# epam/Zstandard

Hardware: AMD Instinct MI355X
Metric: GiB/s compress @ level 3, 64 KiB chunks (higher is better)
Workload: dtype u8; 1 GPU; 4096 independent 65536 B chunks per GPU per step, level 3, BASELINE config[1] shape (Silesia unavailable offline -> Zipf-token log stream, SURVEY 8d); chunks_per_gpu=4096, chunk_bytes=65536, level=3, parallelism=chunks sharded over 1 GPU(s), no collective in the data path

## Files before the change

zstandard_amd/csrc/lz_kernels.hip:

```cpp
#include "zsmi_device.h"
#include "zsmi_scratch.h"
#include <type_traits>

#ifndef ZS_CAND_G
#define ZS_CAND_G 8
#endif
#ifndef ZS_CAND_G_BIG
#define ZS_CAND_G_BIG 16
#endif
#define ZS_CAND_GOF(TLOG) ((TLOG) > ZS_TABLE_LOG_SMALL ? ZS_CAND_G_BIG : ZS_CAND_G)
#ifndef ZS_CAND_DEPTH
#define ZS_CAND_DEPTH 2
#endif
#define ZS_CAND_WAVES(NT) (3 * (NT))
#define ZS_CAND_ROW 65u
#define ZS_CAND_LDS(TLOG, NT) ((size_t)(NT) * (4u << (TLOG)) + 3u * (NT) * ZS_CAND_GOF(TLOG) * ZS_CAND_ROW * 4u + (NT) * 256u + 3u * 16u * 8u + 32u)
#define ZS_SLOT_EMPTY 0xFFFFFFFFu
__device__ __forceinline__ uint32_t zs_hash_short(uint32_t lo, uint32_t hi) { return __umul24(lo, 0x9E3779u) + __umul24(__builtin_amdgcn_alignbit(hi, lo, 16), 0x85EBCBu); }
__device__ __forceinline__ uint32_t zs_hash_long(uint32_t lo, uint32_t hi)
{ return __umul24(lo, 0x9E3779u) + __umul24(__builtin_amdgcn_alignbit(hi, lo, 24), 0x85EBCBu) + __umul24(hi >> 16, 0xC2B2AFu); }

template <int TLOG, int NT, bool PFX = false>
__global__ void __launch_bounds__(64 * ZS_CAND_WAVES(NT))
k_lz_candidates(const uint8_t *__restrict__ src, const ZsUnitDesc *__restrict__ units, uint32_t block0,
                uint16_t *__restrict__ distAll, uint8_t *__restrict__ distHiAll, uint32_t *__restrict__ candCount,
                const ZsCDictEntry *__restrict__ dictTab = nullptr, const uint32_t *__restrict__ unitDict = nullptr,
                const uint32_t *__restrict__ liveUnits = nullptr)
{
    static_assert(!PFX || TLOG == ZS_TABLE_LOG_BIG, "a prefixed unit spans up to 128 KiB of positions");
    if (liveUnits && blockIdx.x >= *liveUnits) return;
    const uint32_t *dictImg = nullptr; uint32_t pfx = 0;
    if constexpr (PFX) {
        const ZsCDictEntry &de = dictTab[unitDict ? unitDict[blockIdx.x] : 0u];
        dictImg = de.img; pfx = (uint32_t)__builtin_amdgcn_readfirstlane((int)de.pfx);
    }
    extern __shared__ __attribute__((aligned(16))) uint32_t candLds[];
    constexpr bool BIG = TLOG > ZS_TABLE_LOG_SMALL;
    constexpr uint32_t G = ZS_CAND_GOF(TLOG), GP = G * 64u, H = G / NT;
    constexpr uint32_t M = ZS_CAND_DEPTH;
    constexpr uint32_t LPS = 64u / G;
    constexpr uint32_t WD = G / 4u + 2u;
    static_assert(G == 8 || G == 16, "a hasher lane takes G consecutive positions of a group: 8 or 16");
    const uint32_t wave = (uint32_t)__builtin_amdgcn_readfirstlane((int)(threadIdx.x >> 6)), lane = threadIdx.x & 63u;
    const uint32_t tab = (wave < NT) ? wave : ((wave < 2 * NT) ? wave - NT : wave - 2 * NT);
    uint32_t *T = candLds + ((size_t)tab << TLOG);
    uint32_t *opnd = candLds + ((size_t)NT << TLOG);
    constexpr uint32_t ROW = ZS_CAND_ROW, GR = G * ROW;
    constexpr uint32_t RING = 3u * NT * GR;
    uint64_t *runMarks = reinterpret_cast<uint64_t *>(opnd + RING + NT * 64u);
    uint32_t *runFlag = opnd + RING + NT * 64u + 3u * 16u * 2u;
    const ZsUnitDesc ud = units[blockIdx.x];
    const uint8_t *s = src + ud.srcOff;
    const uint32_t n = ud.size;
    const size_t slot = (size_t)(ud.firstBlock - block0);
    uint16_t *dist = zs_block_dist(distAll, slot);
    uint8_t *distHi = zs_block_dist_hi(distHiAll, slot);
    const uint32_t hashable = (n >= 8) ? n - 7 : 0;
    const uint32_t nGroups = (hashable + GP - 1) / GP;
    if (threadIdx.x < 2) zs_block_cand(candCount, slot, threadIdx.x) = 0;
    if (nGroups == 0) return;
    if (n >= 16 && (n & 15u) == 0) {
        uint4 f;
        __builtin_memcpy(&f, s, 16);
        const uint32_t splat = (f.x & 0xFFu) * 0x01010101u;
        if (((f.x ^ splat) | (f.y ^ splat) | (f.z ^ splat) | (f.w ^ splat)) == 0) {
            if (threadIdx.x == 0) candLds[0] = 0;
            __syncthreads();
            uint32_t mixed = 0;
            for (uint32_t i = threadIdx.x * 16u; i < n && !mixed; i += ZS_CAND_WAVES(NT) * 64u * 16u) {
                uint4 v;
                __builtin_memcpy(&v, s + i, 16);
                mixed = (v.x ^ splat) | (v.y ^ splat) | (v.z ^ splat) | (v.w ^ splat);
            }
            if (mixed) candLds[0] = 1u;
            __syncthreads();
            const bool uniform = candLds[0] == 0;
            __syncthreads();
            if (uniform) return;
        }
    }
    const uint32_t dummyBase = ((uint32_t)(NT - tab) << TLOG) + RING + tab * 64u;
    auto mergeRead = [&](uint32_t g, uint32_t (&mS)[H], uint32_t (&mL)[H]) {
        const uint32_t *xb = opnd + (size_t)(g % 3u) * NT * GR + (NT > 1 ? tab * H : 0u) * ROW + lane;
        #pragma unroll
        for (uint32_t uu = 0; uu < H; uu++) { mS[uu] = xb[uu * ROW]; mL[uu] = (NT > 1) ? xb[GR + uu * ROW] : 0u; }
    };
    uint32_t found = 0;
    const uint32_t matchlessBelow = n >> ZS_MATCHLESS_SHIFT;
    auto mergeStore = [&](uint32_t g, const uint32_t (&mS)[H], const uint32_t (&mL)[H]) {
        const uint32_t sbase = g * GP + ((NT > 1) ? tab * H * 64u : 0u);
        uint64_t hiMine = 0;
        #pragma unroll
        for (uint32_t uu = 0; uu < H; uu++) {
            const uint32_t dm = (NT > 1) ? (mL[uu] ? mL[uu] : mS[uu]) : mS[uu];
            if (BIG) { const uint64_t hi = __ballot((dm >> 16) != 0); if (lane == uu) hiMine = hi; }
            if (found < matchlessBelow) {
                if ((g + 1u) * GP <= hashable) found += (uint32_t)__popcll(__ballot(dm != 0));
                else found += (uint32_t)__popcll(__ballot(dm != 0 && sbase + uu * 64 + lane < hashable));
            }
            dist[sbase + uu * 64 + lane] = (uint16_t)dm;
        }
        if (BIG && lane < H) *reinterpret_cast<uint64_t *>(distHi + ((sbase + lane * 64) >> 3)) = hiMine;
    };
    if (wave >= 2 * NT) {
        __syncthreads(); __syncthreads();
        for (uint32_t i = 2; i <= nGroups + 1; i++) {
            uint32_t mS[H], mL[H];
            mergeRead(i - 2, mS, mL);
            if (__builtin_amdgcn_readfirstlane((int)runFlag[((i - 2) % 3u) * 2u + tab])) {
                if (lane == 0) runFlag[((i - 2) % 3u) * 2u + tab] = 0;
                #pragma unroll
                for (uint32_t uu = 0; uu < H; uu++) {
                    const uint64_t marks = runMarks[((i - 2) % 3u) * 16u + ((NT > 1) ? tab * H : 0u) + uu];
                    if ((marks >> lane) & 1ull) { if (NT > 1) mL[uu] = 1u; else mS[uu] = 1u; }
                }
            }
            mergeStore(i - 2, mS, mL);
            __syncthreads();
        }
        if (lane == 0) zs_block_cand(candCount, slot, tab) = found;
        return;
    }

    if (wave < NT) {
        if constexpr (PFX) {
            uint4 *t4 = reinterpret_cast<uint4 *>(T);
            const uint4 *img4 = reinterpret_cast<const uint4 *>(dictImg + ((size_t)tab << TLOG));
            #pragma unroll 8
            for (uint32_t i = lane; i < (1u << TLOG) / 4; i += 64) t4[i] = img4[i];
        } else {
            uint4 *t4 = reinterpret_cast<uint4 *>(T);
            const uint4 e = make_uint4(ZS_SLOT_EMPTY, ZS_SLOT_EMPTY, ZS_SLOT_EMPTY, ZS_SLOT_EMPTY);
            #pragma unroll 8
            for (uint32_t i = lane; i < (1u << TLOG) / 4; i += 64) t4[i] = e;
        }
        uint32_t ringSlot = 0;
        __syncthreads();
        for (uint32_t i = 1; i <= nGroups; i++) {
            uint32_t *ob = opnd + ((size_t)ringSlot * NT + tab) * GR + lane;
            const uint32_t base = (i - 1) * GP + lane + (PFX ? pfx : 0u);
            uint32_t op[G], entry[G], old[G];
            #pragma unroll
            for (uint32_t u = 0; u < G; u++) op[u] = ob[u * ROW];
            #pragma unroll
            for (uint32_t u = 0; u < G; u++) {
                uint32_t pu = base + u * 64u;
                asm volatile("" : "+v"(pu));
                entry[u] = (op[u] & 0xFFFE0000u) | pu;
                old[u] = atomicExch(&T[op[u] & 0xFFFFu], entry[u]);
            }
            #pragma unroll
            for (uint32_t u = 0; u < G; u++) {
                const uint32_t x = old[u] ^ entry[u], dd = entry[u] - old[u];
                ob[u * ROW] = (max(x, dd) < (1u << 17)) ? dd : 0u;
            }
            ringSlot = (ringSlot == 2u) ? 0u : ringSlot + 1u;
            __syncthreads();
        }
        __syncthreads();
        return;
    }

    auto run = [&](auto roleTag) {
        constexpr bool LONG = decltype(roleTag)::value;
        const uint32_t stepOfLane = lane / LPS, l0 = (lane % LPS) * G;
        const uint32_t wbase = stepOfLane * ROW + l0;
        const uint32_t last8 = n - 8;
        auto loadGroup = [&](uint32_t g, uint32_t (&w)[WD]) {
            const uint32_t o = g * GP + lane * G;
            #pragma unroll
            for (uint32_t k = 0; k < WD / 2; k++) {
                const uint32_t ok = o + 8u * k, oc = min(ok, last8);
                const uint64_t v = zs_load64(s + oc) >> (8u * min(ok - oc, 7u));
                w[2 * k] = (uint32_t)v; w[2 * k + 1] = (uint32_t)(v >> 32);
            }
        };
        uint32_t bufA[M][WD], bufB[M][WD];
        auto loadM = [&](uint32_t g0, uint32_t (&buf)[M][WD]) {
            #pragma unroll
            for (uint32_t k = 0; k < M; k++) loadGroup(min(g0 + k, nGroups), buf[k]);
        };
        auto iter = [&](auto wholeTag, uint32_t i, const uint32_t (&w)[WD]) {
            constexpr bool WHOLE = decltype(wholeTag)::value;
            const uint32_t ringSlot = i % 3u;
            if (i < nGroups) {
                uint32_t *ob = opnd + ((size_t)ringSlot * NT + tab) * GR + wbase;
                const uint32_t pbase = i * GP + lane * G;
                #pragma unroll
                for (uint32_t u = 0; u < G; u++) {
                    const uint32_t k = u >> 2, sh = u & 3u;
                    const uint32_t lo = sh ? __builtin_amdgcn_alignbyte(w[k + 1], w[k], sh) : w[k];
                    const uint32_t hi = sh ? __builtin_amdgcn_alignbyte(w[min(k + 2, WD - 1)], w[k + 1], sh) : w[k + 1];
                    uint32_t h = LONG ? zs_hash_long(lo, hi) : zs_hash_short(lo, hi);
                    asm volatile("" : "+v"(h));
                    const uint32_t r = __builtin_amdgcn_alignbit(h, h, 32 - TLOG);
                    ob[u] = (WHOLE || pbase + u < hashable) ? (r & (0xFFFE0000u | ((1u << TLOG) - 1u))) : ((r & 0xFFFE0000u) | (dummyBase + l0 + u));
                }
                bool flat = false;
                uint64_t flatLanes = 0;
                if (WHOLE && __ballot(w[0] == w[1])) {
                    uint32_t diff = w[0] ^ __builtin_amdgcn_alignbyte(w[0], w[0], 1);
                    #pragma unroll
                    for (uint32_t k = 1; k < WD; k++) diff |= w[k] ^ w[k - 1];
                    flat = diff == 0;
                    flatLanes = __ballot(flat);
                }
                if (flatLanes) {
                    const uint32_t key = flat ? ((w[0] & 0xFFu) | 0x100u) : 0u;
                    const uint32_t keyBelow = (uint32_t)__builtin_amdgcn_update_dpp(0, (int)key, 0x138, 0xF, 0xF, true);
                    const uint32_t keyAbove = (uint32_t)__builtin_amdgcn_update_dpp(0, (int)key, 0x130, 0xF, 0xF, true);
                    const bool markFirst = flat && keyBelow == key && (lane % LPS) != 0u;
                    const bool innerLast = flat && keyAbove == key && (lane % LPS) != LPS - 1u;
                    if (flat) {
                        uint32_t h = LONG ? zs_hash_long(w[0], w[1]) : zs_hash_short(w[0], w[1]);
                        asm volatile("" : "+v"(h));
                        const uint32_t away = (__builtin_amdgcn_alignbit(h, h, 32 - TLOG) & 0xFFFE0000u) | (dummyBase + l0);
                        if (markFirst) ob[0] = away;
                        #pragma unroll
                        for (uint32_t u = 1; u + 1 < G; u++) ob[u] = away + u;
                        if (innerLast) ob[G - 1] = away + (G - 1);
                    }
                    if (!LONG) {
                        if (lane < NT) runFlag[ringSlot * 2u + lane] = 1u;
                        const uint32_t bits = flat ? (((1u << G) - 2u) | (markFirst ? 1u : 0u)) : 0u;
                        if (G == 8) reinterpret_cast<uint8_t *>(runMarks + ringSlot * 16u)[lane] = (uint8_t)bits;
                        else reinterpret_cast<uint16_t *>(runMarks + ringSlot * 16u)[lane] = (uint16_t)bits;
                    }
                }
            }
            __syncthreads();
        };
        auto step = [&](uint32_t i, const uint32_t (&w)[WD]) {
            if (i > nGroups + 1) return;
            if ((i + 1) * GP + 8u <= n) iter(std::true_type{}, i, w); else iter(std::false_type{}, i, w);
        };
        if (!LONG && lane < 6u) runFlag[lane] = 0;
        loadM(0, bufA);
        for (uint32_t g0 = 0; g0 <= nGroups + 1; g0 += 2 * M) {
            loadM(g0 + M, bufB);
            #pragma unroll
            for (uint32_t k = 0; k < M; k++) step(g0 + k, bufA[k]);
            loadM(g0 + 2 * M, bufA);
            #pragma unroll
            for (uint32_t k = 0; k < M; k++) step(g0 + M + k, bufB[k]);
        }
    };
    if (tab == 0) run(std::false_type{}); else run(std::true_type{});
}

__global__ void __launch_bounds__(1024)
k_lz_dict_tables(const ZsCDictEntry entry, ZsCDictEntry *__restrict__ entryOut)
{
    constexpr int TLOG = ZS_TABLE_LOG_BIG;
    __shared__ uint32_t T[1u << TLOG];
    const uint32_t tab = blockIdx.x, tid = threadIdx.x;
    const uint8_t *__restrict__ pre = entry.pre; const uint32_t pfx = entry.pfx; uint32_t *__restrict__ img = const_cast<uint32_t *>(entry.img);
    if (tab == 0 && tid == 0) *entryOut = entry;
    for (uint32_t i = tid; i < (1u << TLOG); i += 1024) T[i] = 0;
    __syncthreads();
    const uint32_t hashable = pfx >= 8 ? pfx - 7 : 0;
    for (uint32_t p = tid; p < hashable; p += 1024) {
        const uint64_t v = zs_load64(pre + p);
        const uint32_t lo = (uint32_t)v, hi = (uint32_t)(v >> 32);
        const uint32_t h = tab ? zs_hash_long(lo, hi) : zs_hash_short(lo, hi);
        const uint32_t r = __builtin_amdgcn_alignbit(h, h, 32 - TLOG);
        atomicMax(&T[r & ((1u << TLOG) - 1u)], ((p + 1u) << 15) | (r >> 17));
    }
    __syncthreads();
    uint32_t *out = img + ((size_t)tab << TLOG);
    for (uint32_t i = tid; i < (1u << TLOG); i += 1024) {
        const uint32_t k = T[i];
        out[i] = k ? (((k & 0x7FFFu) << 17) | ((k >> 15) - 1u)) : ZS_SLOT_EMPTY;
    }
}

#ifndef ZS_WALK_MINW
#define ZS_WALK_MINW 1
#endif
#define ZS_WALK_WGRP(WLOG) ((WLOG) >= 9 ? 4 : 2)
#ifndef ZS_WALK_LPW_256
#define ZS_WALK_LPW_256 2
#endif
#ifndef ZS_WALK_LPW_512
#define ZS_WALK_LPW_512 4
#endif
#define ZS_WALK_LPW(WLOG) ((WLOG) >= 9 ? ZS_WALK_LPW_512 : ZS_WALK_LPW_256)
#define ZS_WALK_THREADS(BIG, WLOG) ((((BIG) ? ZS_UNIT_MAX : ZS_BLOCK_MAX) >> (WLOG)) * ZS_WALK_LPW(WLOG))
#define ZS_WALK_KERNEL(LOOK, REPW, BIG, WLOG) k_lz_walk<ZS_WALK_LPW(WLOG), ZS_WALK_WGRP(WLOG), LOOK, REPW, BIG, ZS_WALK_THREADS(BIG, WLOG)>
#ifndef ZS_WALK_SKEW
#define ZS_WALK_SKEW  24u
#endif
#define ZS_WALK_FRONT 48u
#define ZS_WALK_TAIL  144u
#define ZS_WALK_SRCBYTES(CAPB) ((((CAPB) + ZS_WALK_TAIL + ZS_WALK_SKEW * (((CAPB) + ZS_WALK_TAIL) / 256u + 1u)) + 15u) & ~15u)
#define ZS_WALK_LDS(CAPB) ((CAPB) / 8 + 16 + ZS_WALK_FRONT + ZS_WALK_SRCBYTES(CAPB) + 16 + 1024)

typedef const __attribute__((address_space(3))) uint32_t *ZsLdsU32;
template <int K>
__device__ __forceinline__ void lds_span(uint32_t byteOff, uint32_t (&out)[K])
{
    ZsLdsU32 d = (ZsLdsU32)(uintptr_t)(byteOff & ~3u);
    uint32_t w[K + 1];
    #pragma unroll
    for (int k = 0; k <= K; k++) w[k] = d[k];
    const uint32_t sh = byteOff & 3u;
    #pragma unroll
    for (int k = 0; k < K; k++) out[k] = __builtin_amdgcn_alignbyte(w[k + 1], w[k], sh);
}
template <int I, int K>
__device__ __forceinline__ uint32_t span_at(const uint32_t (&v)[K])
{
    if constexpr ((I & 3) == 0) return v[I >> 2];
    else return __builtin_amdgcn_alignbyte(v[(I >> 2) + 1], v[I >> 2], I & 3);
}
__device__ __forceinline__ uint32_t zs_agree16(const uint32_t (&a)[4], const uint32_t (&b)[4])
{
    const uint64_t x0 = (uint64_t)(a[0] ^ b[0]) | ((uint64_t)(a[1] ^ b[1]) << 32), x1 = (uint64_t)(a[2] ^ b[2]) | ((uint64_t)(a[3] ^ b[3]) << 32);
    const uint32_t n0 = x0 ? ((uint32_t)__builtin_ctzll(x0) >> 3) : 8u;
    const uint32_t n1 = x1 ? ((uint32_t)__builtin_ctzll(x1) >> 3) : 8u;
    return (n0 < 8u) ? n0 : 8u + n1;
}
template <int LPW> __device__ __forceinline__ uint32_t walker_or(uint32_t v)
{
    if constexpr (LPW >= 2) v |= (uint32_t)__builtin_amdgcn_update_dpp(0, (int)v, 0xB1, 0xF, 0xF, false);
    if constexpr (LPW == 4) v |= (uint32_t)__builtin_amdgcn_update_dpp(0, (int)v, 0x4E, 0xF, 0xF, false);
    return v;
}
template <int LPW> __device__ __forceinline__ int walker_max(int v)
{
    if constexpr (LPW >= 2) v = max(v, __builtin_amdgcn_update_dpp(0, v, 0xB1, 0xF, 0xF, false));
    if constexpr (LPW == 4) v = max(v, __builtin_amdgcn_update_dpp(0, v, 0x4E, 0xF, 0xF, false));
    return v;
}
template <int LPW> __device__ __forceinline__ uint32_t walker_min(uint32_t v)
{
    if constexpr (LPW >= 2) v = min(v, (uint32_t)__builtin_amdgcn_update_dpp(0, (int)v, 0xB1, 0xF, 0xF, false));
    if constexpr (LPW == 4) v = min(v, (uint32_t)__builtin_amdgcn_update_dpp(0, (int)v, 0x4E, 0xF, 0xF, false));
    return v;
}
template <int NT, int DIR>
__device__ __forceinline__ uint32_t block_scan_max(uint32_t v, uint32_t *wv, uint32_t tid, uint32_t *total)
{
    const uint32_t lane = tid & 63u, wave = tid >> 6;
    #pragma unroll
    for (int d = 1; d < 64; d <<= 1) {
        const uint32_t o = (uint32_t)(DIR > 0 ? __shfl_up((int)v, d) : __shfl_down((int)v, d));
        if (DIR > 0 ? (int)lane >= d : (int)lane + d < 64) v = max(v, o);
    }
    __syncthreads();
    if (lane == (DIR > 0 ? 63u : 0u)) wv[wave] = v;
    __syncthreads();
    uint32_t pre = 0, all = 0;
    #pragma unroll
    for (uint32_t k = 0; k < NT / 64; k++) { const uint32_t x = wv[k]; all = max(all, x); if (DIR > 0 ? k < wave : k > wave) pre = max(pre, x); }
    *total = all;
    return max(v, pre);
}
__device__ __forceinline__ uint32_t zs_nonzero8(const uint4 d)
{
    typedef uint16_t u16x2 __attribute__((ext_vector_type(2)));
    const u16x2 one = { 1, 1 };
    (void)one;
    auto nz = [&](uint32_t w) { uint32_t r; asm("v_pk_min_u16 %0, %1, %2" : "=v"(r) : "v"(w), "v"(0x00010001u)); return r; };
    const uint32_t v = nz(d.x) | (nz(d.y) << 2) | (nz(d.z) << 4) | (nz(d.w) << 6);
    return (v | (v >> 15)) & 0xFFu;
}

#ifdef ZS_WALK_PROFILE
#define WPROF_STAMP(k) { __builtin_amdgcn_sched_barrier(0); unsigned long long t_; asm volatile("s_waitcnt vmcnt(0) lgkmcnt(0)\n\ts_memtime %0\n\ts_waitcnt lgkmcnt(0)" : "=s"(t_) :: "memory"); __builtin_amdgcn_sched_barrier(0); wprof[k] += t_ - wlast; wlast = t_; }
#else
#define WPROF_STAMP(k)
#endif
#define ZS_WALK_KERNEL_PFX(LOOK, REPW, WLOG) k_lz_walk<ZS_WALK_LPW(WLOG), ZS_WALK_WGRP(WLOG), LOOK, REPW, true, ZS_WALK_THREADS(false, WLOG), true>
template <int LPW, int WGRP, int LOOK, int REPWIN, bool BIG, int NT, bool PFX = false>
__global__ void __launch_bounds__(NT, BIG ? 1 : ZS_WALK_MINW)
k_lz_walk(const uint8_t *__restrict__ src, const ZsUnitDesc *__restrict__ units, uint32_t block0,
          const uint16_t *__restrict__ distAll, const uint8_t *__restrict__ distHiAll,
          uint2 *__restrict__ recAll, uint32_t junkSlot, uint4 *__restrict__ resAll, int rangeLogArg, const uint32_t *__restrict__ candCount,
          const ZsCDictEntry *__restrict__ dictTab = nullptr, const uint32_t *__restrict__ unitDict = nullptr,
          const uint32_t *__restrict__ liveUnits = nullptr)
{
    static_assert(!PFX || BIG, "a prefixed unit is staged in the 128 KiB layout");
    if (liveUnits && blockIdx.x >= *liveUnits) return;
    const uint8_t *pre = nullptr; uint32_t pfx = 0;
    if constexpr (PFX) {
        const ZsCDictEntry &de = dictTab[unitDict ? unitDict[blockIdx.x] : 0u];
        pre = de.pre; pfx = (uint32_t)__builtin_amdgcn_readfirstlane((int)de.pfx);
    }
    constexpr uint32_t CAP = BIG ? ZS_UNIT_MAX : ZS_BLOCK_MAX;
    constexpr uint32_t CPL = LOOK / LPW, RPL = REPWIN / LPW, GPL = WGRP / LPW;
    static_assert((LPW == 1 || LPW == 2 || LPW == 4) && WGRP % LPW == 0 && LOOK % LPW == 0 && REPWIN % LPW == 0 && CPL >= 1 && RPL >= 1 && LOOK <= 8 && REPWIN <= 8, "a walker's lanes share the groups and candidates evenly");
    static_assert(NT >= 64 && NT % 64 == 0 && NT * GPL * 16 <= CAP / 8, "the exchange buffer holds 16 bytes a lane and group");
    extern __shared__ __attribute__((aligned(16))) uint8_t walkLds[];
    constexpr uint32_t SRC = CAP / 8 + 16 + ZS_WALK_FRONT;
    auto lposv = [](uint32_t v) { return SRC + v + (uint32_t)__mul24((int)v >> 8, (int)ZS_WALK_SKEW); };
    const uint32_t vb = PFX ? pfx : 0u;
    auto lpos = [&](uint32_t p) { return lposv(p + vb); };
    auto stage16 = [&](uint32_t i, const uint4 v) {
        uint8_t *d = walkLds + lposv(i);
        *reinterpret_cast<uint2 *>(d) = make_uint2(v.x, v.y); *reinterpret_cast<uint2 *>(d + 8) = make_uint2(v.z, v.w);
        const uint32_t o = i & 255u;
        if (o == 0) { *reinterpret_cast<uint2 *>(d - ZS_WALK_SKEW) = make_uint2(v.x, v.y); *reinterpret_cast<uint2 *>(d - ZS_WALK_SKEW + 8) = make_uint2(v.z, v.w); }
        else if (o == 16) *reinterpret_cast<uint2 *>(d - ZS_WALK_SKEW) = make_uint2(v.x, v.y);
    };
    const uint32_t tid = threadIdx.x, lane = tid & 63u;
    const uint32_t rangeLog = (uint32_t)rangeLogArg, R = 1u << rangeLog;
    const ZsUnitDesc ud = units[blockIdx.x];
    const uint32_t slot = ud.firstBlock - block0;
    const uint8_t *s = src + ud.srcOff;
    const uint32_t n = ud.size;
    const uint16_t *dist = zs_block_dist(distAll, slot);
    const uint8_t *distHi = zs_block_dist_hi(distHiAll, slot);
    uint4 *xbuf = reinterpret_cast<uint4 *>(walkLds);
    const uint32_t xw = (tid & ~63u) * GPL;
    const uint32_t safeAddr = (xw + lane) * 16u;
    uint32_t *queue = reinterpret_cast<uint32_t *>(walkLds + SRC + ZS_WALK_SRCBYTES(CAP));
    uint4 *res = zs_block_range_results(resAll, slot);
    uint8_t *xhi = reinterpret_cast<uint8_t *>(queue + 4);
    uint2 *recs = zs_block_walk_records(recAll, slot);
    const uint32_t sub = lane & (LPW - 1u);
#ifdef ZS_WALK_PROFILE
    unsigned long long wprof[10] = { 0, 0, 0, 0, 0, 0, 0, 0, 0, 0 }, wlast;
    asm volatile("s_memtime %0\n\ts_waitcnt lgkmcnt(0)" : "=s"(wlast) :: "memory");
#endif

    if (zs_block_cand(candCount, slot, 0) + zs_block_cand(candCount, slot, 1) < (n >> ZS_MATCHLESS_SHIFT)) {
        const uint32_t nRanges = (n + R - 1) >> rangeLog, perBlockLog = 16u - rangeLog;
        for (uint32_t r = tid; r < nRanges; r += NT) res[zs_unit_range_result(r, perBlockLog)] = make_uint4(0, 0, 0, 0);
        return;
    }
    uint32_t mixed = 0;
    if (tid < (ZS_WALK_FRONT - ZS_WALK_SKEW) / 4) reinterpret_cast<uint32_t *>(walkLds + SRC - ZS_WALK_FRONT)[tid] = 0;
    if (tid == 0) { queue[0] = 0; queue[1] = 0; }
    __syncthreads();
    if constexpr (PFX) {
        const uint32_t end = pfx + n, splat = (n ? (uint32_t)s[0] : 0u) * 0x01010101u;
        for (uint32_t i = tid * 16; i < end + ZS_WALK_TAIL && i + 16 <= CAP + ZS_WALK_TAIL; i += NT * 16) {
            uint4 w = make_uint4(0, 0, 0, 0);
            if (i + 16 <= pfx) __builtin_memcpy(&w, pre + i, 16);
            else if (i >= pfx && i + 16 <= end) {
                __builtin_memcpy(&w, s + (i - pfx), 16);
                mixed |= (w.x ^ splat) | (w.y ^ splat) | (w.z ^ splat) | (w.w ^ splat);
            } else if (i < end) {
                uint8_t b[16];
                for (uint32_t k = 0; k < 16; k++) {
                    const uint32_t v = i + k;
                    b[k] = v < pfx ? pre[v] : (v < end ? s[v - pfx] : (uint8_t)0);
                    if (v >= pfx && v < end && b[k] != (uint8_t)splat) mixed = 1;
                }
                __builtin_memcpy(&w, b, 16);
            }
            stage16(i, w);
        }
        if ((n & 15u) != 0 || n < 16) mixed = 1;
    } else {
        constexpr uint32_t PER = (CAP / 16 + NT - 1) / NT;
        const uint32_t nFull = n & ~15u;
        uint4 v[PER];
        const uint32_t splat = (n ? (uint32_t)s[0] : 0u) * 0x01010101u;
        #pragma unroll
        for (uint32_t k = 0; k < PER; k++) {
            const uint32_t i = (tid + k * NT) * 16;
            const uint32_t ii = (i + 16 <= nFull) ? i : 0u;
            v[k] = make_uint4(0, 0, 0, 0);
            if (nFull >= 16) __builtin_memcpy(&v[k], s + ii, 16);
        }
        #pragma unroll
        for (uint32_t k = 0; k < PER; k++) {
            const uint32_t i = (tid + k * NT) * 16;
            if (i + 16 <= nFull) stage16(i, v[k]);
            mixed |= (v[k].x ^ splat) | (v[k].y ^ splat) | (v[k].z ^ splat) | (v[k].w ^ splat);
        }
        if (n != nFull || n < 16) mixed = 1;
        for (uint32_t i = nFull + tid * 16; i < n + ZS_WALK_TAIL; i += NT * 16) {
            uint4 w = make_uint4(0, 0, 0, 0);
            if (i < n) {
                uint64_t lo = 0, hi = 0;
                for (uint32_t k = 0; k < 16 && i + k < n; k++) { const uint64_t c = s[i + k]; if (k < 8) lo |= c << (8 * k); else hi |= c << (8 * (k - 8)); }
                w = make_uint4((uint32_t)lo, (uint32_t)(lo >> 32), (uint32_t)hi, (uint32_t)(hi >> 32));
            }
            if (i + 16 <= CAP + ZS_WALK_TAIL) stage16(i, w);
        }
    }
#if defined(ZS_WALK_STOP) && ZS_WALK_STOP == 1
    if (n) return;
#endif
    const uint32_t hashable = (n >= 8) ? n - 7 : 0;
    if (mixed) queue[1] = 1u;
    __syncthreads();
    if (queue[1] == 0) {
        const uint32_t nRanges = (n + R - 1) >> rangeLog, perBlockLog = 16u - rangeLog;
        for (uint32_t r = tid; r < nRanges; r += NT) res[zs_unit_range_result(r, perBlockLog)] = make_uint4(0, 0, 0, 0);
        return;
    }
    WPROF_STAMP(0)

    {
        const uint32_t nRanges = (n + R - 1) >> rangeLog;
        bool active = false, more = true;
        uint32_t r = 0, ip = 0, anchor = 0, scanEnd = 0, limit = 0, rep0 = 0, rep1 = 0, nseq = 0, lastOff = 0, recBase = 0, blockBase = 0;
        uint2 heldRec = make_uint2(0, 0);
        const uint32_t perBlockLog = 16u - rangeLog;
        auto resIndex = [&](uint32_t rr) { return zs_unit_range_result(rr, perBlockLog); };
        typedef __attribute__((address_space(3))) uint4 *ZsLdsU4;
        const uint32_t xwaveLds = (uint32_t)__builtin_amdgcn_readfirstlane((int)(uint32_t)(uintptr_t)(ZsLdsU4)(xbuf + xw));
        uint32_t gh[GPL] = {};
        auto loadGroup = [&](uint32_t p) {
            #pragma unroll
            for (uint32_t k = 0; k < GPL; k++) {
                const uint32_t g = (p >> 3) + sub + LPW * k;
                const uint16_t *gsrc = dist + (size_t)g * 8u;
                uint32_t keep;
                asm volatile("s_mov_b32 %0, m0\n\ts_mov_b32 m0, %2\n\ts_nop 0\n\tglobal_load_lds_dwordx4 %1, off\n\ts_mov_b32 m0, %0" : "=&s"(keep) : "v"(gsrc), "s"(xwaveLds + k * 1024u) : "memory");
                if (BIG) gh[k] = (uint32_t)distHi[g];
            }
        };
        for (;;) {
            if (__any(!active && more)) {
                const uint64_t idle = __ballot(!active && more && sub == 0);
                uint32_t base = 0;
                if (lane == 0) base = atomicAdd(queue, (uint32_t)__popcll(idle));
                base = (uint32_t)__builtin_amdgcn_readfirstlane((int)base);
                if (!active && more) {
                    const uint32_t leader = lane & ~(LPW - 1u);
                    r = base + (uint32_t)__popcll(idle & ((1ull << leader) - 1ull));
                    if (r >= nRanges) more = false;
                    else {
                        const uint32_t start = r << rangeLog;
                        const uint32_t blockStart = start & ~(ZS_BLOCK_MAX - 1);
                        const uint32_t blockEnd = blockStart + min(n - blockStart, ZS_BLOCK_MAX);
                        const uint32_t end = min(start + R, blockEnd);
                        limit = min(end + ZS_CROSS_MAX, blockEnd);
                        scanEnd = (blockEnd - blockStart >= 16) ? min(end, hashable) : 0;
                        ip = start; anchor = start; rep0 = 0; rep1 = 0; nseq = 0; lastOff = 0; recBase = start >> 2; blockBase = blockStart;
                        active = ip < scanEnd;
                        if (!active && sub == 0) res[resIndex(r)] = make_uint4(0, 0, 0, 0);
                        if (active) { loadGroup(ip); asm volatile("s_waitcnt vmcnt(0)" ::: "memory"); }
                    }
                }
            }
            if (!__any(active)) { if (!__any(more)) break; continue; }
            WPROF_STAMP(1)
#ifdef ZS_WALK_PROFILE
            wprof[8] += 1; wprof[9] += (unsigned long long)__popcll(__ballot(active));
#endif
            const uint32_t wend = min((ip & ~7u) + 8u * WGRP, scanEnd);
            uint32_t rm0 = 0, rm1 = 0;
            {
                const bool t0 = active && rep0 != 0 && ip + vb >= rep0, t1 = active && rep1 != 0 && ip + vb >= rep1;
                const uint32_t p0 = ip + sub * RPL;
                constexpr int SP = (RPL + 3 + 3) / 4;
                uint32_t a[SP] = {}, b[SP] = {}, c[SP] = {};
                {
                    const bool tr = t0 || t1;
                    lds_span<SP>(tr ? lpos(p0) : safeAddr, a);
                    lds_span<SP>(tr ? lpos(t0 ? p0 - rep0 : p0) : safeAddr, b);
                    lds_span<SP>(tr ? lpos(t1 ? p0 - rep1 : p0) : safeAddr, c);
                }
                auto tryAt = [&](auto iTag) {
                    constexpr int I = decltype(iTag)::value;
                    const uint32_t q = p0 + I;
                    const bool ok = q < wend && q + 4 <= limit;
                    const uint32_t av = span_at<I>(a);
                    if (t0 && ok && av == span_at<I>(b)) rm0 |= 1u << (sub * RPL + I);
                    if (t1 && ok && av == span_at<I>(c)) rm1 |= 1u << (sub * RPL + I);
                };
                tryAt(std::integral_constant<int, 0>{});
                if constexpr (RPL >= 2) tryAt(std::integral_constant<int, 1>{});
                if constexpr (RPL >= 4) { tryAt(std::integral_constant<int, 2>{}); tryAt(std::integral_constant<int, 3>{}); }
                if constexpr (RPL >= 8) { tryAt(std::integral_constant<int, 4>{}); tryAt(std::integral_constant<int, 5>{}); tryAt(std::integral_constant<int, 6>{}); tryAt(std::integral_constant<int, 7>{}); }
                rm0 = walker_or<LPW>(rm0); rm1 = walker_or<LPW>(rm1);
                rm1 &= ~rm0;
            }
            WPROF_STAMP(2)
            asm volatile("s_waitcnt vmcnt(0)" ::: "memory");
            uint32_t m = 0;
            #pragma unroll
            for (uint32_t k = 0; k < GPL; k++) {
                const uint4 gd = xbuf[xw + 64u * k + lane];
                if (BIG) xhi[xw + 64u * k + lane] = (uint8_t)gh[k];
                m |= (zs_nonzero8(gd) | gh[k]) << (8u * (sub + LPW * k));
            }
            m = walker_or<LPW>(m) >> (ip & 7u);
            if (active) m = (m & (0xFFFFFFFFu >> (32u - (wend - ip)))) | rm0 | rm1; else m = 0;
            {
                const uint32_t skip = sub * CPL;
                if constexpr ((LPW - 1) * CPL >= 4) { uint32_t t = m & (m - 1); t &= t - 1; t &= t - 1; t &= t - 1; m = (skip & 4u) ? t : m; }
                if constexpr ((((LPW - 1) * CPL) & 2) != 0 || (LPW == 4 && CPL == 2)) { uint32_t t = m & (m - 1); t &= t - 1; m = (skip & 2u) ? t : m; }
                if constexpr ((CPL & 1) != 0) { const uint32_t t = m & (m - 1); m = (skip & 1u) ? t : m; }
            }
            uint32_t idx[CPL], off[CPL], dv[CPL]; bool have[CPL], isRep[CPL];
            #pragma unroll
            for (uint32_t c = 0; c < CPL; c++) {
                have[c] = m != 0;
                idx[c] = have[c] ? (uint32_t)__builtin_ctz(m) : 0u;
                m &= m - 1;
                const uint32_t q = ip + idx[c];
                const uint32_t j = (q >> 3) - (ip >> 3);
                const uint32_t owner = xw + 64u * (j / LPW) + (lane & ~(LPW - 1u)) + (j % LPW);
                dv[c] = reinterpret_cast<const uint16_t *>(xbuf + owner)[q & 7u];
                if (BIG) dv[c] |= (((uint32_t)xhi[owner] >> (q & 7u)) & 1u) << 16;
            }
            #pragma unroll
            for (uint32_t c = 0; c < CPL; c++) asm volatile("" : "+v"(dv[c]));
            #pragma unroll
            for (uint32_t c = 0; c < CPL; c++) {
                const bool r0 = ((rm0 >> idx[c]) & 1u) != 0, r1 = ((rm1 >> idx[c]) & 1u) != 0;
                isRep[c] = have[c] && (r0 || r1);
                off[c] = r0 ? rep0 : (r1 ? rep1 : dv[c]);
                if (!have[c]) off[c] = 0;
            }
            WPROF_STAMP(3)
            int bestKey = 0; uint32_t bestPack = 0, bestOff = 0;
            uint32_t sa[CPL][3], sb[CPL][3];
            #pragma unroll
            for (uint32_t c = 0; c < CPL; c++) {
                const uint32_t q = ip + idx[c];
                #pragma unroll
                for (int k = 0; k < 3; k++) { sa[c][k] = 0; sb[c][k] = 0; }
                const bool tr = have[c];
                lds_span<3>(tr ? lpos(q - 4) : safeAddr, sa[c]);
                lds_span<3>(tr ? lpos(q - off[c] - 4) : safeAddr, sb[c]);
            }
            #pragma unroll
            for (uint32_t c = 0; c < CPL; c++) asm volatile("" : "+v"(sa[c][0]), "+v"(sa[c][1]), "+v"(sa[c][2]), "+v"(sb[c][0]), "+v"(sb[c][1]), "+v"(sb[c][2]));
            #pragma unroll
            for (uint32_t c = 0; c < CPL; c++) {
                const uint32_t q = ip + idx[c];
                const uint32_t (&a)[3] = sa[c], (&b)[3] = sb[c];
                const uint32_t xb = a[0] ^ b[0], x0 = a[1] ^ b[1], x1 = a[2] ^ b[2];
                const uint32_t f0 = x0 ? (uint32_t)__builtin_ctz(x0) : 32u, f1 = x1 ? (uint32_t)__builtin_ctz(x1) : 32u;
                const uint32_t fwd = min(((x0 ? f0 : 32u + f1)) >> 3, limit - q);
                const uint32_t maxBack = min(min(q - anchor, q + vb - off[c]), ZS_BCAP);
                const uint32_t back = min(xb ? ((uint32_t)__builtin_clz(xb) >> 3) : 4u, maxBack);
                if (have[c] && fwd >= (isRep[c] ? ZS_REPMIN : ZS_MINMATCH)) {
                    const int gain = (int)(4u * fwd + 8u * back) - (isRep[c] ? 0 : (int)zs_highbit(off[c] + 1)) - 5 * (int)idx[c];
                    const int key = ((gain + 2048) << 3) | (int)(7u - (sub * CPL + c));
                    if (key > bestKey) { bestKey = key; bestPack = idx[c] | (fwd << 8) | (back << 16); bestOff = off[c]; }
                }
            }
            const int best = walker_max<LPW>(bestKey);
            const bool took = active && best != 0;
            const uint32_t packed = walker_or<LPW>(bestKey == best ? bestPack : 0u), boff = walker_or<LPW>(bestKey == best ? bestOff : 0u);
            const uint32_t bq = ip + (packed & 0xFFu), bback = packed >> 16;
            uint32_t bfwd = (packed >> 8) & 0xFFu;
            WPROF_STAMP(4)
            const bool extend = took && bfwd == ZS_FCAP && (limit - bq) > ZS_FCAP;
            bool need = extend;
            uint32_t pos = bq + ZS_FCAP;
            while (__any(need)) {
                uint32_t e = 0xFFFFFFFFu;
                if (need) {
                    const uint32_t cap = limit - pos, fo = 16u * sub;
                    uint32_t nb = 0;
                    if (fo < cap) {
                        uint32_t a[4], b[4];
                        lds_span<4>(lpos(pos + fo), a);
                        lds_span<4>(lpos(pos - boff + fo), b);
                        nb = zs_agree16(a, b);
                    }
                    if (nb < 16u || fo + 16u >= cap) e = min(fo + nb, cap);
                }
                e = walker_min<LPW>(e);
                if (need) {
                    if (e != 0xFFFFFFFFu) { pos += e; need = false; }
                    else pos += 16u * LPW;
                }
            }
            if (extend) bfwd = pos - bq;
            WPROF_STAMP(5)
            uint32_t recLl = 0;
            if (took) {
                recLl = bq - bback - anchor;
                nseq++; lastOff = boff;
                ip = bq + bfwd; anchor = ip;
                if (boff == rep1) { rep1 = rep0; rep0 = boff; }
                else if (boff != rep0) { rep1 = rep0; rep0 = boff; }
            } else if (active) ip = wend;
            if (took) {
                const uint2 rec = make_uint2((bq - bback - blockBase) | ((bback + bfwd) << 17), boff | (recLl << 17));
                if (nseq & 1u) heldRec = rec;
                else if (sub == 0) *reinterpret_cast<uint4 *>(recs + recBase + nseq - 2) = make_uint4(heldRec.x, heldRec.y, rec.x, rec.y);
            }
            if (active && ip >= scanEnd) {
                if (sub == 0) {
                    if (nseq & 1u) recs[recBase + nseq - 1] = heldRec;
                    res[resIndex(r)] = make_uint4(nseq, nseq ? anchor - blockBase : 0u, lastOff, 0u);
                }
                active = false;
            }
            if (active) loadGroup(ip);
            WPROF_STAMP(6)
        }
    }
    WPROF_STAMP(1)
#ifdef ZS_WALK_PROFILE
    __syncthreads();
    if (lane == 0) { unsigned long long *o = zs_res_lend_walk_profile(resAll, junkSlot) + ((size_t)blockIdx.x * (NT / 64) + (tid >> 6)) * 10; for (int k = 0; k < 10; k++) o[k] = wprof[k]; }
#endif
}

__global__ void __launch_bounds__(256)
k_lz_stitch(const ZsBlockDesc *__restrict__ blocks, const uint2 *__restrict__ recAll, const uint4 *__restrict__ resAll,
            ZsSeqRec *__restrict__ seqAll, uint32_t *__restrict__ hdrAll, int rangeLogArg, const uint32_t *__restrict__ liveBlocks = nullptr)
{
    constexpr int NT = 256;
    if (liveBlocks && blockIdx.x >= *liveBlocks) return;
    __shared__ __attribute__((aligned(16))) uint32_t sa[4 * 256 + 16];
    uint32_t *sKept = sa, *sStart = sa + 256, *sWave = sa + 1024, *sTot = sa + 1028, *sMl = sa + 1032, *sEnd = sa + 1036;
    uint2 *sInfo = reinterpret_cast<uint2 *>(sa + 512);
    const uint32_t tid = threadIdx.x, lane = tid & 63u;
    const uint32_t rangeLog = (uint32_t)rangeLogArg;
    const uint32_t slot = blockIdx.x;
    const uint32_t NRB = ZS_BLOCK_MAX >> rangeLog;
    const uint2 *recs = zs_block_walk_records(recAll, slot);
    const uint4 *res = zs_block_range_results(resAll, slot);
    {
        const uint32_t bStart = 0, bi = 0;
        const uint32_t bN = blocks[slot].size;
        const uint32_t bEnd = bN;
        const uint32_t t = tid;
        const bool mine = t < NRB;
        const bool walked = mine && bN >= 16 && (t << rangeLog) < bN;
        const uint4 rr = walked ? res[t] : make_uint4(0, 0, 0, 0);
        const uint32_t ns = rr.x, le = rr.y;
        const uint32_t rs = min(bStart + (t << rangeLog), bEnd);
        const uint2 *rp = recs + ((bStart + (t << rangeLog)) >> 2);
        uint32_t total;
        const uint32_t key = ns ? ((le << 9) | (511u - t)) : 0u;
        const uint32_t incl = block_scan_max<NT, 1>(key, sWave, tid, &total);
        uint32_t excl = (uint32_t)__shfl_up((int)incl, 1);
        if (lane == 0) { excl = 0; for (uint32_t k = 0; k < (tid >> 6); k++) excl = max(excl, sWave[k]); }
        const uint32_t own = max(excl >> 9, bStart), reachAll = max(total >> 9, bStart);
        const uint32_t definer = 511u - (excl & 511u);
#if defined(ZS_STITCH_STOP) && ZS_STITCH_STOP == 2
        if (bN) return;
#endif
        uint32_t f = 0, fStart = 0, fEnd = 0, fOff = 0;
        if (ns && own >= rs) {
            if (le <= own) f = ns;
            else {
                const uint4 r01 = *reinterpret_cast<const uint4 *>(rp);
                auto endOf = [](uint32_t x) { return (x & 0x1FFFFu) + (x >> 17); };
                uint2 rec = make_uint2(r01.x, r01.y), nxt = make_uint2(r01.z, r01.w);
                bool haveNxt = ns > 1;
                if (endOf(r01.x) > own) f = 0;
                else if (ns > 1 && endOf(r01.z) > own) { f = 1; rec = nxt; haveNxt = false; }
                else {
                    uint32_t lo = 2, hi = ns - 1;
                    while (lo < hi) { const uint32_t mid = (lo + hi) >> 1; if (endOf(rp[mid].x) > own) hi = mid; else lo = mid + 1; }
                    f = lo; rec = rp[f]; haveNxt = false;
                }
                uint32_t st = rec.x & 0x1FFFFu, en = endOf(rec.x);
                if (st < own && en - own < ZS_MINMATCH) {
                    f++;
                    if (f < ns) { rec = haveNxt ? nxt : rp[f]; st = rec.x & 0x1FFFFu; en = endOf(rec.x); }
                }
                fStart = max(st, own); fEnd = en; fOff = rec.y & 0x1FFFFu;
            }
        }
        const bool keptAny = f < ns;
        sKept[t] = (keptAny ? 1u : 0u) | (rr.z << 1);
        __syncthreads();
        const uint32_t defWord = sKept[excl != 0 ? definer : 0u];
        const bool joined = keptAny && excl != 0 && own >= rs && fStart == own && fOff == (defWord >> 1) && (defWord & 1u) != 0;
        const uint32_t fOut = f + (joined ? 1u : 0u), cnt = ns - fOut;
        const bool stopper = ns && le > own && !(joined && cnt == 0);
        uint32_t total2;
        const uint32_t key2 = stopper ? (((512u - t) << 18) | (joined ? fEnd : own)) : 0u;
        const uint32_t sfx = block_scan_max<NT, -1>(key2, sWave, tid, &total2);
        uint32_t sfxEx = (uint32_t)__shfl_down((int)sfx, 1);
        if (lane == 63) { sfxEx = 0; for (uint32_t k = (tid >> 6) + 1; k < NT / 64; k++) sfxEx = max(sfxEx, sWave[k]); }
        const uint32_t chainEnd = sfxEx ? (sfxEx & 0x3FFFFu) : reachAll;
        const uint32_t wave = tid >> 6;
        const uint32_t cntIncl = wave_incl_scan(cnt);
        if (lane == 63) sTot[wave] = cntIncl;
        sInfo[t] = make_uint2(own | (fOut << 17), chainEnd | (ns << 17));
        __syncthreads();
        uint32_t start = cntIncl - cnt, nseq = 0;
        #pragma unroll
        for (uint32_t k = 0; k < NT / 64; k++) { const uint32_t x = sTot[k]; nseq += x; if (k < wave) start += x; }
        sStart[t] = start;
        __syncthreads();
#if defined(ZS_STITCH_STOP) && ZS_STITCH_STOP == 1
        if (bN) return;
#endif
        constexpr uint32_t PB = 4;
        ZsSeqRec *out = zs_block_seqs(seqAll, slot);
        uint2 recN[PB]; uint32_t ownN[PB], endN[PB];
        auto request = [&](uint32_t base) {
            #pragma unroll
            for (uint32_t q = 0; q < PB; q++) {
                const uint32_t d = base + NT * q + tid;
                recN[q] = make_uint2(0, 0); ownN[q] = 0; endN[q] = 0;
                if (d < nseq) {
                    uint32_t jr = 0;
                    #pragma unroll
                    for (uint32_t stepb = NT / 2; stepb >= 1; stepb >>= 1) if (d >= sStart[jr + stepb]) jr += stepb;
                    const uint2 info = sInfo[jr];
                    const uint32_t at = d - sStart[jr], k = (info.x >> 17) + at;
                    ownN[q] = (info.x & 0x1FFFFu) | (at == 0 ? 0x80000000u : 0u);
                    endN[q] = (info.y & 0x1FFFFu) | (k + 1 == (info.y >> 17) ? 0x80000000u : 0u);
                    recN[q] = recs[(jr << (rangeLog - 2)) + k];
                }
            }
        };
        request(0);
        #pragma unroll
        for (uint32_t q = 0; q < PB; q++) asm volatile("" : "+v"(recN[q].x), "+v"(recN[q].y));
        uint32_t mlSum = 0;
        for (uint32_t base = 0; base < nseq; base += NT * PB) {
            uint2 recC[PB]; uint32_t ownC[PB], endC[PB];
            #pragma unroll
            for (uint32_t q = 0; q < PB; q++) { recC[q] = recN[q]; ownC[q] = ownN[q]; endC[q] = endN[q]; }
            if (base + NT * PB < nseq) request(base + NT * PB);
            #pragma unroll
            for (uint32_t q = 0; q < PB; q++) {
                const uint32_t d = base + NT * q + tid;
                if (d < nseq) {
                    const uint2 rec = recC[q];
                    uint32_t st = rec.x & 0x1FFFFu, ml = rec.x >> 17;
                    const uint32_t off = rec.y & 0x1FFFFu, en = st + ml;
                    if (ownC[q] >> 31) {
                        const uint32_t ownj = ownC[q] & 0x1FFFFu;
                        if (st < ownj) { st = ownj; ml = en - st; }
                    }
                    if (endC[q] >> 31) ml = (endC[q] & 0x1FFFFu) - st;
                    ZsSeqRec w; w.x = zs_rec_x(ml, off); w.y = zs_rec_y(off, st);
                    out[d] = w;
                    mlSum += ml;
                    if (d + 1 == nseq) sEnd[0] = st + ml;
                }
            }
        }
        const uint32_t mlWave = wave_sum(mlSum);
        if (lane == 0) sMl[wave] = mlWave;
        __syncthreads();
        if (tid == 0) {
            uint32_t covered = 0;
            for (uint32_t k = 0; k < NT / 64; k++) covered += sMl[k];
            ZsBlockHdr h; h.nseq = nseq; h.trailing = bN - (nseq ? sEnd[0] : 0u); h.lits = bN - covered; h.pad = 0;
            zs_block_hdr(hdrAll, slot) = h;
        }
    }
}
```

Measured before the change: 147.5 GiB/s.

## Assign walk ranges statically per walker instead of an LDS atomic work queue

Replaces the dynamic LDS atomic queue that handed out walk ranges with a fixed mapping of one range per walker group (tid/LPW), guarded by a static_assert that the thread count covers a full-capacity unit. M0 is set once outside the loop, and the per-load M0 save and restore is dropped when GPL is 1. The record and rep-offset update logic is rewritten with selects instead of branches. This removes the atomic, ballot and readfirstlane overhead per range and reduces divergence, but gives up dynamic load balancing, so slow ranges can no longer be offset by walkers picking up more work.

```diff
diff --git a/zstandard_amd/csrc/lz_kernels.hip b/zstandard_amd/csrc/lz_kernels.hip
--- a/zstandard_amd/csrc/lz_kernels.hip
+++ b/zstandard_amd/csrc/lz_kernels.hip
@@ -286,6 +286,9 @@
 #endif
 #define ZS_WALK_LPW(WLOG) ((WLOG) >= 9 ? ZS_WALK_LPW_512 : ZS_WALK_LPW_256)
 #define ZS_WALK_THREADS(BIG, WLOG) ((((BIG) ? ZS_UNIT_MAX : ZS_BLOCK_MAX) >> (WLOG)) * ZS_WALK_LPW(WLOG))
+static_assert(ZS_WALK_THREADS(false, 8) / ZS_WALK_LPW(8) == (ZS_BLOCK_MAX >> 8) && ZS_WALK_THREADS(false, 9) / ZS_WALK_LPW(9) == (ZS_BLOCK_MAX >> 9) &&
+              ZS_WALK_THREADS(true, 8) / ZS_WALK_LPW(8) == (ZS_UNIT_MAX >> 8) && ZS_WALK_THREADS(true, 9) / ZS_WALK_LPW(9) == (ZS_UNIT_MAX >> 9),
+              "a walker per walk range of a unit of full capacity");
 #define ZS_WALK_KERNEL(LOOK, REPW, BIG, WLOG) k_lz_walk<ZS_WALK_LPW(WLOG), ZS_WALK_WGRP(WLOG), LOOK, REPW, BIG, ZS_WALK_THREADS(BIG, WLOG)>
 #ifndef ZS_WALK_SKEW
 #define ZS_WALK_SKEW  24u
@@ -414,9 +417,9 @@
     uint4 *xbuf = reinterpret_cast<uint4 *>(walkLds);
     const uint32_t xw = (tid & ~63u) * GPL;
     const uint32_t safeAddr = (xw + lane) * 16u;
-    uint32_t *queue = reinterpret_cast<uint32_t *>(walkLds + SRC + ZS_WALK_SRCBYTES(CAP));
+    uint32_t *mixedWord = reinterpret_cast<uint32_t *>(walkLds + SRC + ZS_WALK_SRCBYTES(CAP)) + 1;
     uint4 *res = zs_block_range_results(resAll, slot);
-    uint8_t *xhi = reinterpret_cast<uint8_t *>(queue + 4);
+    uint8_t *xhi = reinterpret_cast<uint8_t *>(mixedWord + 3);
     uint2 *recs = zs_block_walk_records(recAll, slot);
     const uint32_t sub = lane & (LPW - 1u);
 #ifdef ZS_WALK_PROFILE
@@ -431,7 +434,7 @@
     }
     uint32_t mixed = 0;
     if (tid < (ZS_WALK_FRONT - ZS_WALK_SKEW) / 4) reinterpret_cast<uint32_t *>(walkLds + SRC - ZS_WALK_FRONT)[tid] = 0;
-    if (tid == 0) { queue[0] = 0; queue[1] = 0; }
+    if (tid == 0) *mixedWord = 0;
     __syncthreads();
     if constexpr (PFX) {
         const uint32_t end = pfx + n, splat = (n ? (uint32_t)s[0] : 0u) * 0x01010101u;
@@ -486,9 +489,9 @@
     if (n) return;
 #endif
     const uint32_t hashable = (n >= 8) ? n - 7 : 0;
-    if (mixed) queue[1] = 1u;
+    if (mixed) *mixedWord = 1u;
     __syncthreads();
-    if (queue[1] == 0) {
+    if (*mixedWord == 0) {
         const uint32_t nRanges = (n + R - 1) >> rangeLog, perBlockLog = 16u - rangeLog;
         for (uint32_t r = tid; r < nRanges; r += NT) res[zs_unit_range_result(r, perBlockLog)] = make_uint4(0, 0, 0, 0);
         return;
@@ -497,49 +500,40 @@
 
     {
         const uint32_t nRanges = (n + R - 1) >> rangeLog;
-        bool active = false, more = true;
-        uint32_t r = 0, ip = 0, anchor = 0, scanEnd = 0, limit = 0, rep0 = 0, rep1 = 0, nseq = 0, lastOff = 0, recBase = 0, blockBase = 0;
+        bool active = false;
+        uint32_t ip = 0, anchor = 0, scanEnd = 0, limit = 0, rep0 = 0, rep1 = 0, nseq = 0, lastOff = 0, blockBase = 0;
         uint2 heldRec = make_uint2(0, 0);
         const uint32_t perBlockLog = 16u - rangeLog;
-        auto resIndex = [&](uint32_t rr) { return zs_unit_range_result(rr, perBlockLog); };
         typedef __attribute__((address_space(3))) uint4 *ZsLdsU4;
         const uint32_t xwaveLds = (uint32_t)__builtin_amdgcn_readfirstlane((int)(uint32_t)(uintptr_t)(ZsLdsU4)(xbuf + xw));
+        asm volatile("s_mov_b32 m0, %0\n\ts_nop 0" :: "s"(xwaveLds) : "memory");
         uint32_t gh[GPL] = {};
         auto loadGroup = [&](uint32_t p) {
             #pragma unroll
             for (uint32_t k = 0; k < GPL; k++) {
                 const uint32_t g = (p >> 3) + sub + LPW * k;
                 const uint16_t *gsrc = dist + (size_t)g * 8u;
-                uint32_t keep;
-                asm volatile("s_mov_b32 %0, m0\n\ts_mov_b32 m0, %2\n\ts_nop 0\n\tglobal_load_lds_dwordx4 %1, off\n\ts_mov_b32 m0, %0" : "=&s"(keep) : "v"(gsrc), "s"(xwaveLds + k * 1024u) : "memory");
+                if constexpr (GPL == 1) asm volatile("global_load_lds_dwordx4 %0, off" :: "v"(gsrc) : "memory");
+                else asm volatile("s_mov_b32 m0, %1\n\ts_nop 0\n\tglobal_load_lds_dwordx4 %0, off" :: "v"(gsrc), "s"(xwaveLds + k * 1024u) : "memory");
                 if (BIG) gh[k] = (uint32_t)distHi[g];
             }
         };
-        for (;;) {
-            if (__any(!active && more)) {
-                const uint64_t idle = __ballot(!active && more && sub == 0);
-                uint32_t base = 0;
-                if (lane == 0) base = atomicAdd(queue, (uint32_t)__popcll(idle));
-                base = (uint32_t)__builtin_amdgcn_readfirstlane((int)base);
-                if (!active && more) {
-                    const uint32_t leader = lane & ~(LPW - 1u);
-                    r = base + (uint32_t)__popcll(idle & ((1ull << leader) - 1ull));
-                    if (r >= nRanges) more = false;
-                    else {
-                        const uint32_t start = r << rangeLog;
-                        const uint32_t blockStart = start & ~(ZS_BLOCK_MAX - 1);
-                        const uint32_t blockEnd = blockStart + min(n - blockStart, ZS_BLOCK_MAX);
-                        const uint32_t end = min(start + R, blockEnd);
-                        limit = min(end + ZS_CROSS_MAX, blockEnd);
-                        scanEnd = (blockEnd - blockStart >= 16) ? min(end, hashable) : 0;
-                        ip = start; anchor = start; rep0 = 0; rep1 = 0; nseq = 0; lastOff = 0; recBase = start >> 2; blockBase = blockStart;
-                        active = ip < scanEnd;
-                        if (!active && sub == 0) res[resIndex(r)] = make_uint4(0, 0, 0, 0);
-                        if (active) { loadGroup(ip); asm volatile("s_waitcnt vmcnt(0)" ::: "memory"); }
-                    }
-                }
-            }
-            if (!__any(active)) { if (!__any(more)) break; continue; }
+        const uint32_t r = tid / LPW;
+        const uint32_t recBase = r << (rangeLog - 2u), resAt = zs_unit_range_result(r, perBlockLog);
+        if (r < nRanges) {
+            const uint32_t start = r << rangeLog;
+            const uint32_t blockStart = start & ~(ZS_BLOCK_MAX - 1);
+            const uint32_t blockEnd = blockStart + min(n - blockStart, ZS_BLOCK_MAX);
+            const uint32_t end = min(start + R, blockEnd);
+            limit = min(end + ZS_CROSS_MAX, blockEnd);
+            scanEnd = (blockEnd - blockStart >= 16) ? min(end, hashable) : 0;
+            ip = start; anchor = start; blockBase = blockStart;
+            active = ip < scanEnd;
+            if (!active && sub == 0) res[resAt] = make_uint4(0, 0, 0, 0);
+            if (active) loadGroup(ip);
+        }
+        asm volatile("s_waitcnt vmcnt(0)" ::: "memory");
+        while (__any(active)) {
             WPROF_STAMP(1)
 #ifdef ZS_WALK_PROFILE
             wprof[8] += 1; wprof[9] += (unsigned long long)__popcll(__ballot(active));
@@ -669,26 +663,20 @@
             }
             if (extend) bfwd = pos - bq;
             WPROF_STAMP(5)
-            uint32_t recLl = 0;
-            if (took) {
-                recLl = bq - bback - anchor;
-                nseq++; lastOff = boff;
-                ip = bq + bfwd; anchor = ip;
-                if (boff == rep1) { rep1 = rep0; rep0 = boff; }
-                else if (boff != rep0) { rep1 = rep0; rep0 = boff; }
-            } else if (active) ip = wend;
-            if (took) {
-                const uint2 rec = make_uint2((bq - bback - blockBase) | ((bback + bfwd) << 17), boff | (recLl << 17));
-                if (nseq & 1u) heldRec = rec;
-                else if (sub == 0) *reinterpret_cast<uint4 *>(recs + recBase + nseq - 2) = make_uint4(heldRec.x, heldRec.y, rec.x, rec.y);
-            }
-            if (active && ip >= scanEnd) {
-                if (sub == 0) {
-                    if (nseq & 1u) recs[recBase + nseq - 1] = heldRec;
-                    res[resIndex(r)] = make_uint4(nseq, nseq ? anchor - blockBase : 0u, lastOff, 0u);
-                }
-                active = false;
-            }
+            const uint32_t recStart = bq - bback, recLl = recStart - anchor;
+            const uint2 rec = make_uint2((recStart - blockBase) | ((bback + bfwd) << 17), boff | (recLl << 17));
+            const bool rot = took && boff != rep0;
+            rep1 = rot ? rep0 : rep1; rep0 = rot ? boff : rep0;
+            nseq += took ? 1u : 0u;
+            lastOff = took ? boff : lastOff;
+            ip = took ? bq + bfwd : (active ? wend : ip);
+            anchor = took ? ip : anchor;
+            const bool odd = (nseq & 1u) != 0, done = active && ip >= scanEnd, first = sub == 0;
+            if (took && !odd && first) *reinterpret_cast<uint4 *>(recs + recBase + nseq - 2) = make_uint4(heldRec.x, heldRec.y, rec.x, rec.y);
+            heldRec.x = (took && odd) ? rec.x : heldRec.x; heldRec.y = (took && odd) ? rec.y : heldRec.y;
+            if (done && odd && first) recs[recBase + nseq - 1] = heldRec;
+            if (done && first) res[resAt] = make_uint4(nseq, nseq ? anchor - blockBase : 0u, lastOff, 0u);
+            active = active && !done;
             if (active) loadGroup(ip);
             WPROF_STAMP(6)
         }
```

Result: faster. 149.8 GiB/s, median of 6 (+1.6%).
